# TtesseractT/Synthetic-Audio-Detection

Measured on AMD Instinct MI355X. Metric: 4s@32kHz segments/sec end-to-end (mel+ResNet+ensemble), 1/2/4/8 MI355X, higher is better.
Workload: dtype bf16; 1 GPU; end-to-end inference: B int16 4 s segments resident in HBM -> mel front end -> ResNet-18@512x512 -> 6 binary heads -> merge (+RCCL all-gather of logits); heads=6, distinct_backbones=1, micro_batch=2048, parallelism=dp1, frontend_overlapped=True

## Files before the change

synthetic-audio-detection_amd/csrc/l2conv.hip:

```cpp
#include "common.hpp"
#include "igemm.hpp"
#include "kernels.hpp"
#include "rwconv.hpp"

namespace sad {

namespace l2c {
constexpr int NW = 4;
constexpr int PW = 18, PR = PW * PW;
constexpr int NDP = (PR + 7) / 8;
constexpr int PATCH = NDP * 1024;
constexpr int ROWB = PW * 128;
constexpr int QP = (NDP + NW - 1) / NW;
constexpr int RESB = 256 * 256;
constexpr int NRP = RESB / 1024 / NW;
constexpr int NDS = 256 * 128 / 1024 / NW;
constexpr int OFF_RES = 2 * PATCH;
constexpr int SMEM_RES = OFF_RES + RESB;
constexpr int NS = 36;
constexpr int NSC = 18;
constexpr int DQ = 4;
constexpr int WV = 8;
constexpr int BAD = 0x7FFFFFF0;
constexpr uint64_t KEY = 0xd92dad912240ull;
constexpr int TABB = NW * QP * 256;
constexpr int TAIL = 512 + TABB;
constexpr int ESH = 27;
static_assert(SMEM_RES + TAIL <= 160 * 1024, "LDS budget");
static_assert(PATCH % 128 == 0 && OFF_RES % 256 == 0, "buffer offsets commute with the chunk XORs");
}

__device__ __forceinline__ int l2c_key(int x) { return (int)((l2c::KEY >> (3 * x)) & 7); }

template <bool RES, bool DS, bool X3, bool ST, bool AB>
__device__ __forceinline__ void l2conv_body(const BlockConvArgs& a) {
  static_assert(!(RES && DS) && !(X3 && DS), "one shortcut form");
  static_assert(!ST || (!RES && !DS && !X3), "statistics: the plain bf16 form");
  static_assert(!AB || (!X3 && !ST), "ablations: the bf16 forms");
  using namespace l2c;
  constexpr int TP = X3 ? 8 : 16;
  constexpr int UPT = 2 * TP;
  constexpr int NUC = 9 * UPT;
  constexpr int PDIV = X3 ? 8 : 16;
  constexpr int DQ = X3 ? 8 : l2c::DQ;
  constexpr int OFF_B = RES || DS ? SMEM_RES : OFF_RES;
  constexpr int OFF_T = OFF_B + 512;
  extern __shared__ __attribute__((aligned(256))) char smem[];
  const int tid = threadIdx.x, lane = tid & 63;
  const int wave = __builtin_amdgcn_readfirstlane(tid >> 6);
  const int fr = lane & 15, fg = lane >> 4;
  const int ab = AB ? a.ablate : 0;
  const int cw = X3 ? (wave & 1) * 32 : wave * 32;
  const int r0w = X3 ? (wave >> 1) * 8 : 0;
  const int w = xcd_remap(blockIdx.x, gridDim.x);
  const int tiles_x = a.W / 16, tiles_img = tiles_x * (a.H / 16);
  const int tiles_p = a.N * tiles_img;
  const int tp_begin = (int)((int64_t)w * tiles_p / gridDim.x), tp_end = (int)((int64_t)(w + 1) * tiles_p / gridDim.x);
  if (tp_begin >= tp_end) {
    if constexpr (ST) a.st_part[(int64_t)w * 256 + tid] = 0.f;
    return;
  }

  l1b_v4 rx = {(unsigned)(uintptr_t)a.in0, (unsigned)((uintptr_t)a.in0 >> 32) & 0xFFFFu, (unsigned)a.in0_bytes, 0x00020000u};
  asm volatile("" : "+s"(rx));
  const void* const rrp = RES ? (const void*)a.res : (const void*)a.in1;
  l1b_v4 rr = {(unsigned)(uintptr_t)rrp, (unsigned)((uintptr_t)rrp >> 32) & 0xFFFFu,
               (unsigned)(RES ? a.res_bytes : a.in1_bytes), 0x00020000u};
  if constexpr (RES || DS) asm volatile("" : "+s"(rr));
  const __amdgpu_buffer_rsrc_t ro =
      __builtin_amdgcn_make_buffer_rsrc((void*)a.out, (short)0, (int)a.out_bytes, 0x00020000);
  const unsigned lds0 = (unsigned)(uintptr_t)(__attribute__((address_space(3))) char*)smem;
  const int ps = (int)a.in0_pstride * 2;
  const int pso = (int)a.out_pstride * 2;
  const int pss = RES ? (int)a.res_pstride * 2 : DS ? a.ss1 * (int)a.in1_pstride * 2 : 0;
  const int srow = RES ? a.W * pss : DS ? a.ss1 * a.W1 * (int)a.in1_pstride * 2 : 0;
  const int orow = a.W * pso;

  struct TileO {
    int base, oy0, ox0, sbase, obase;
  };
  auto tile_o = [&](int t) __attribute__((always_inline)) {
    const int b = t / tiles_img, rem = t - b * tiles_img;
    const int ty = rem / tiles_x;
    TileO o;
    o.oy0 = ty * 16;
    o.ox0 = (rem - ty * tiles_x) * 16;
    o.base = ((b * a.H + o.oy0) * a.W + o.ox0) * ps;
    o.obase = ((b * a.H + o.oy0) * a.W + o.ox0) * pso;
    o.sbase = RES  ? ((b * a.H + o.oy0) * a.W + o.ox0) * pss
              : DS ? ((b * a.H1 + o.oy0 * a.ss1) * a.W1 + o.ox0 * a.ss1) * (int)(a.in1_pstride * 2)
                   : 0;
    return o;
  };
  const int wrap_i = 15 * a.W * ps, wrap_o = 15 * orow, wrap_s = 16 * srow - a.W * pss;
  auto tile_step = [&](const TileO& o) __attribute__((always_inline)) {
    TileO n;
    n.ox0 = o.ox0 + 16;
    n.oy0 = o.oy0;
    n.base = o.base + 16 * ps;
    n.obase = o.obase + 16 * pso;
    n.sbase = o.sbase + 16 * pss;
    if (n.ox0 == a.W) {
      n.ox0 = 0;
      n.oy0 += 16;
      n.base += wrap_i;
      n.obase += wrap_o;
      n.sbase += wrap_s;
      if (n.oy0 == a.H) n.oy0 = 0;
    }
    return n;
  };

  const int TA = (int)lds0 + OFF_T + (wave * (QP * 64) + lane) * 4;
  auto piece_entry = [&](int k) __attribute__((always_inline)) {
    const int r = 8 * (wave + NW * k) + (lane >> 3);
    const int Y = (r * 3641) >> 16, X = r - PW * Y;
    const int edge = (r >= PR ? 1 : 0) | (Y == 0 ? 2 : 0) | (Y == PW - 1 ? 4 : 0) | (X == 0 ? 8 : 0) | (X == PW - 1 ? 16 : 0);
    const unsigned off = (unsigned)((Y * a.W + X) * ps + (((lane & 7) ^ l2c_key(X)) << 4)) >> 4;
    return (int)(((unsigned)edge << ESH) | (off & ((1u << ESH) - 1)));
  };
  auto patch_base = [&](const TileO& o) __attribute__((always_inline)) { return o.base - (a.W + 1) * ps; };
  auto patch_mask = [&](const TileO& o) __attribute__((always_inline)) {
    return (int)((unsigned)(1 | (o.oy0 == 0 ? 2 : 0) | (o.oy0 + 16 == a.H ? 4 : 0) | (o.ox0 == 0 ? 8 : 0) |
                            (o.ox0 + 16 == a.W ? 16 : 0))
                 << ESH);
  };
  const unsigned dstw = __builtin_amdgcn_readfirstlane(lds0 + wave * 1024);
  auto issue_piece = [&](auto kc, auto cc, int e, int pbase, int pmask) __attribute__((always_inline)) {
    constexpr int k = decltype(kc)::value, c = decltype(cc)::value;
    if constexpr (NW * k + NW - 1 >= NDP)
      if (wave + NW * k >= NDP) return;
    l1b_dma16<c * PATCH + k * NW * 1024>(rx, (e & pmask) ? BAD : pbase + (int)((unsigned)e << 4), dstw);
  };
  const int pxr = 4 * wave + (lane >> 4);
  const int RV = pxr * pss + (((lane & 15) ^ pxr) << 4);
  auto issue_res = [&](auto kc, const TileO& o) __attribute__((always_inline)) {
    constexpr int k = decltype(kc)::value;
    l1b_dma16<OFF_RES + k * NW * 1024>(rr, RV + (o.sbase + k * srow), dstw);
  };
  const int pxd = 8 * (wave & 1) + (lane >> 3);
  const int DV = (wave >> 1) * srow + pxd * pss + (((lane & 7) ^ ((pxd >> 1) & 7)) << 4);
  auto issue_ds = [&](auto kc, const TileO& o) __attribute__((always_inline)) {
    constexpr int k = decltype(kc)::value;
    l1b_dma16<OFF_RES + k * NW * 1024>(rr, DV + (o.sbase + 2 * k * srow), dstw);
  };
  l1b_v4 wds[2][2];
  if constexpr (DS) {
#pragma unroll
    for (int i = 0; i < 2; ++i)
#pragma unroll
      for (int h = 0; h < 2; ++h)
        wds[i][h] = *(const l1b_v4*)((const u16*)a.wt + (size_t)(cw + 16 * i + fr) * a.wt_ld + 9 * 128 + (fg + 4 * h) * 8);
  }

  l1b_v4 wr[2][NS];
#pragma unroll
  for (int i = 0; i < 2; ++i)
#pragma unroll
    for (int s = 0; s < NS; ++s) {
      const int c = s / NSC, tap = (s % NSC) >> 1, h = s & 1;
      wr[i][s] = *(const l1b_v4*)((const u16*)a.wt + (size_t)(cw + 16 * i + fr) * a.wt_ld + tap * 128 + c * 64 +
                                  (fg + 4 * h) * 8);
    }
  if (tid < (X3 ? 16 : 32)) *(float4*)(smem + OFF_B + 16 * tid) = *(const float4*)(a.bias + 4 * tid);
  TileO ocur = tile_o(tp_begin);
  l1b_for<QP>([&](auto kc) __attribute__((always_inline)) {
    constexpr int k = decltype(kc)::value;
    const int e = piece_entry(k);
    l1b_st<int>(TA + 256 * k, e);
    issue_piece(kc, std::integral_constant<int, 0>{}, e, patch_base(ocur), patch_mask(ocur));
  });

  int I2[3];
#pragma unroll
  for (int kx = 0; kx < 3; ++kx)
    I2[kx] = (int)lds0 + r0w * ROWB + (fr + kx) * 128 + ((fg ^ l2c_key(fr + kx)) << 4);
  const int BA = (int)lds0 + OFF_B + (cw + fg * 4) * 4;
  const int OV = ((r0w + (fg & 1)) * a.W + fr) * pso + ((X3 ? 64 * (cw >> 5) : cw) + (fg >> 1) * 8) * 2;
  const int RB = (int)lds0 + OFF_RES + (r0w * 16 + fr) * 256 + ((((X3 ? 8 * (cw >> 5) : cw >> 3) + (fg >> 1)) ^ fr) << 4) +
                 (fg & 1) * 8;
  const int DD = (int)lds0 + OFF_RES + fr * 128 + ((fg ^ ((fr >> 1) & 7)) << 4);
  const int rl = a.relu ? 0 : (int)0x80008000u;
  const bool relu = a.relu;

  asm volatile("s_waitcnt vmcnt(0)" ::: "memory");
  __syncthreads();
  f32x4 acc[2][TP];
#pragma unroll
  for (int i = 0; i < 2; ++i) {
    const f32x4 b0 = l1b_ld<f32x4>(BA + 64 * i);
#pragma unroll
    for (int j = 0; j < TP; ++j) acc[i][j] = b0;
  }

  float st_s[2][4] = {}, st_q[2][4] = {};
  for (int t = tp_begin; t < tp_end; ++t) {
    const TileO ostep = tile_step(ocur);
    const TileO onext = t + 1 < tp_end ? ostep : ocur;
    const TileO o = ocur;
    const int pb1 = patch_base(o) + 128, pm1 = patch_mask(o);
    const int pb0n = patch_base(onext), pm0n = patch_mask(onext);

    l1b_for<2>([&](auto cc) __attribute__((always_inline)) {
      constexpr int c = decltype(cc)::value;
      if constexpr (c == 0)
        asm volatile("s_waitcnt vmcnt(16)" ::: "memory");
      else
        asm volatile("s_waitcnt vmcnt(0)" ::: "memory");
      __builtin_amdgcn_s_barrier();
      asm volatile("" ::: "memory");
      int pe = l1b_ld<int>(TA);
      int I2c[3][2];
#pragma unroll
      for (int kx = 0; kx < 3; ++kx) {
        I2c[kx][0] = I2[kx] + c * PATCH;
        I2c[kx][1] = I2c[kx][0] ^ 64;
      }
      auto rd = [&](auto uc) __attribute__((always_inline)) -> l1b_v4 {
        constexpr int u = decltype(uc)::value;
        constexpr int tap = u / UPT, ky = tap / 3, kx = tap % 3;
        constexpr int j = X3 ? (u % UPT) / 2 : u % 16, h = X3 ? u % 2 : (u % UPT) / 16;
        return l1b_ld<l1b_v4>(I2c[kx][h] + (j + ky) * ROWB);
      };
      l1b_v4 bq[DQ];
      l1b_for<DQ>([&](auto uc) __attribute__((always_inline)) { bq[decltype(uc)::value] = rd(uc); });
      l1b_for<NUC>([&](auto uc) __attribute__((always_inline)) {
        constexpr int u = decltype(uc)::value;
        constexpr int tap = u / UPT;
        constexpr int j = X3 ? (u % UPT) / 2 : u % 16, h = X3 ? u % 2 : (u % UPT) / 16;
        constexpr int s = c * NSC + 2 * tap + h;
        constexpr int s_hi = c * NSC + 2 * tap, s_lo = s_hi + 1;
        const l1b_v4 bf = bq[u % DQ];
        if constexpr (u + DQ < NUC) bq[u % DQ] = rd(std::integral_constant<int, u + DQ>{});
        if constexpr (u % PDIV == 0 && u / PDIV < QP) {
          constexpr int k = u / PDIV;
          if (!(ab & 32))
            issue_piece(std::integral_constant<int, k>{}, std::integral_constant<int, c ^ 1>{}, pe, c == 0 ? pb1 : pb0n,
                        c == 0 ? pm1 : pm0n);
          if constexpr (k + 1 < QP) pe = l1b_ld<int>(TA + 256 * (k + 1));
        }
        if constexpr (RES && c == 0 && u % PDIV == PDIV / 2 && u / PDIV < NRP)
          issue_res(std::integral_constant<int, u / PDIV>{}, o);
        if constexpr (DS && c == 0 && u % 32 == 8 && u / 32 < NDS) issue_ds(std::integral_constant<int, u / 32>{}, o);
        auto mm = [&](auto ic, auto sc) __attribute__((always_inline)) {
          constexpr int i = decltype(ic)::value, ss = decltype(sc)::value;
          if constexpr (i == 1 && ss >= NS - WV)
            l1b_mfma_v(acc[i][j], wr[i][ss], bf);
          else
            l1b_mfma_a(acc[i][j], wr[i][ss], bf);
        };
        if constexpr (!X3) {
          mm(std::integral_constant<int, 0>{}, std::integral_constant<int, s>{});
          mm(std::integral_constant<int, 1>{}, std::integral_constant<int, s>{});
        } else if constexpr (u == NUC - 2) {
          const l1b_v4 xl = bq[(u + 1) % DQ];
          static_assert(j == TP - 1 && h == 0, "last fragment");
          if constexpr (s_hi >= NS - WV)
            asm volatile(
                "v_mfma_f32_16x16x32_bf16 %0, %2, %6, %0\n\t"
                "v_mfma_f32_16x16x32_bf16 %1, %3, %6, %1\n\t"
                "v_mfma_f32_16x16x32_bf16 %0, %4, %6, %0\n\t"
                "v_mfma_f32_16x16x32_bf16 %1, %5, %6, %1\n\t"
                "v_mfma_f32_16x16x32_bf16 %0, %2, %7, %0\n\t"
                "v_mfma_f32_16x16x32_bf16 %1, %3, %7, %1\n\t"
                "s_nop 11"
                : "+v"(acc[0][j]), "+v"(acc[1][j])
                : "a"(wr[0][s_hi]), "v"(wr[1][s_hi]), "a"(wr[0][s_lo]), "v"(wr[1][s_lo]), "v"(bf), "v"(xl));
          else
            asm volatile(
                "v_mfma_f32_16x16x32_bf16 %0, %2, %6, %0\n\t"
                "v_mfma_f32_16x16x32_bf16 %1, %3, %6, %1\n\t"
                "v_mfma_f32_16x16x32_bf16 %0, %4, %6, %0\n\t"
                "v_mfma_f32_16x16x32_bf16 %1, %5, %6, %1\n\t"
                "v_mfma_f32_16x16x32_bf16 %0, %2, %7, %0\n\t"
                "v_mfma_f32_16x16x32_bf16 %1, %3, %7, %1\n\t"
                "s_nop 11"
                : "+v"(acc[0][j]), "+v"(acc[1][j])
                : "a"(wr[0][s_hi]), "a"(wr[1][s_hi]), "a"(wr[0][s_lo]), "a"(wr[1][s_lo]), "v"(bf), "v"(xl));
        } else if constexpr (u == NUC - 1) {
        } else if constexpr (h == 0) {
          mm(std::integral_constant<int, 0>{}, std::integral_constant<int, s_hi>{});
          mm(std::integral_constant<int, 1>{}, std::integral_constant<int, s_hi>{});
          mm(std::integral_constant<int, 0>{}, std::integral_constant<int, s_lo>{});
          mm(std::integral_constant<int, 1>{}, std::integral_constant<int, s_lo>{});
        } else {
          mm(std::integral_constant<int, 0>{}, std::integral_constant<int, s_hi>{});
          mm(std::integral_constant<int, 1>{}, std::integral_constant<int, s_hi>{});
        }
      });
    });
    if constexpr (DS) {
      constexpr int DQD = 8;
      const int DD1 = DD ^ 64;
      auto rdd = [&](auto uc) __attribute__((always_inline)) -> l1b_v4 {
        constexpr int u = decltype(uc)::value;
        return l1b_ld<l1b_v4>((u / 16 ? DD1 : DD) + (u % 16) * 16 * 128);
      };
      l1b_v4 bd[DQD];
      l1b_for<DQD>([&](auto uc) __attribute__((always_inline)) { bd[decltype(uc)::value] = rdd(uc); });
      l1b_for<32>([&](auto uc) __attribute__((always_inline)) {
        constexpr int u = decltype(uc)::value, h = u / 16, j = u % 16;
        const l1b_v4 bf = bd[u % DQD];
        if constexpr (u + DQD < 32) bd[u % DQD] = rdd(std::integral_constant<int, u + DQD>{});
        l1b_mfma_v(acc[0][j], wds[0][h], bf);
        l1b_mfma_v(acc[1][j], wds[1][h], bf);
      });
    }
    __builtin_amdgcn_sched_barrier(0);
    asm volatile("s_nop 11" ::: "memory");
    __builtin_amdgcn_sched_barrier(0);
    f32x4 bv[2];
#pragma unroll
    for (int i = 0; i < 2; ++i) bv[i] = l1b_ld<f32x4>(BA + 64 * i);

#pragma unroll
    for (int j = 0; j < TP; j += 2) {
      const int osj = o.obase + j * orow;
#pragma unroll
      for (int i = 0; i < 2; ++i) {
        f32x4 v0 = acc[i][j], v1 = acc[i][j + 1];
        const int rbi = i ? RB ^ 32 : RB;
        if constexpr (X3) {
          if constexpr (RES) {
            const l1b_v2 h0 = l1b_ld<l1b_v2>(rbi + j * 4096);
            const l1b_v2 l0 = l1b_ld<l1b_v2>((rbi ^ 64) + j * 4096);
            const l1b_v2 h1 = l1b_ld<l1b_v2>(rbi + (j + 1) * 4096);
            const l1b_v2 l1 = l1b_ld<l1b_v2>((rbi ^ 64) + (j + 1) * 4096);
            v0[0] += __uint_as_float(h0.x << 16) + __uint_as_float(l0.x << 16);
            v0[1] += __uint_as_float(h0.x & 0xFFFF0000u) + __uint_as_float(l0.x & 0xFFFF0000u);
            v0[2] += __uint_as_float(h0.y << 16) + __uint_as_float(l0.y << 16);
            v0[3] += __uint_as_float(h0.y & 0xFFFF0000u) + __uint_as_float(l0.y & 0xFFFF0000u);
            v1[0] += __uint_as_float(h1.x << 16) + __uint_as_float(l1.x << 16);
            v1[1] += __uint_as_float(h1.x & 0xFFFF0000u) + __uint_as_float(l1.x & 0xFFFF0000u);
            v1[2] += __uint_as_float(h1.y << 16) + __uint_as_float(l1.y << 16);
            v1[3] += __uint_as_float(h1.y & 0xFFFF0000u) + __uint_as_float(l1.y & 0xFFFF0000u);
          }
          if (relu)
#pragma unroll
            for (int r = 0; r < 4; ++r) {
              v0[r] = fmaxf(v0[r], 0.f);
              v1[r] = fmaxf(v1[r], 0.f);
            }
          uint32_t qh[4] = {l1b_pk(v0[0], v0[1]), l1b_pk(v0[2], v0[3]), l1b_pk(v1[0], v1[1]), l1b_pk(v1[2], v1[3])};
          const float vv[8] = {v0[0], v0[1], v0[2], v0[3], v1[0], v1[1], v1[2], v1[3]};
          uint32_t ql[4];
#pragma unroll
          for (int e = 0; e < 4; ++e)
            ql[e] = l1b_pk(vv[2 * e] - __uint_as_float(qh[e] << 16), vv[2 * e + 1] - __uint_as_float(qh[e] & 0xFFFF0000u));
#pragma unroll
          for (int e = 0; e < 2; ++e) {
            const auto rh = __builtin_amdgcn_permlane16_swap(qh[e], qh[e + 2], false, false);
            qh[e] = rh[0];
            qh[e + 2] = rh[1];
            const auto rl2 = __builtin_amdgcn_permlane16_swap(ql[e], ql[e + 2], false, false);
            ql[e] = rl2[0];
            ql[e + 2] = rl2[1];
          }
          __builtin_amdgcn_raw_buffer_store_b128((l1b_v4){qh[0], qh[1], qh[2], qh[3]}, ro, OV + 32 * i, osj, 0);
          __builtin_amdgcn_raw_buffer_store_b128((l1b_v4){ql[0], ql[1], ql[2], ql[3]}, ro, OV + 32 * i + 64, osj, 0);
          acc[i][j] = bv[i];
          acc[i][j + 1] = bv[i];
          continue;
        }
        if constexpr (RES) {
          const l1b_v2 r0 = l1b_ld<l1b_v2>(rbi + j * 4096);
          const l1b_v2 r1 = l1b_ld<l1b_v2>(rbi + (j + 1) * 4096);
          v0[0] += __uint_as_float(r0.x << 16);
          v0[1] += __uint_as_float(r0.x & 0xFFFF0000u);
          v0[2] += __uint_as_float(r0.y << 16);
          v0[3] += __uint_as_float(r0.y & 0xFFFF0000u);
          v1[0] += __uint_as_float(r1.x << 16);
          v1[1] += __uint_as_float(r1.x & 0xFFFF0000u);
          v1[2] += __uint_as_float(r1.y << 16);
          v1[3] += __uint_as_float(r1.y & 0xFFFF0000u);
        }
        if constexpr (ST) {
#pragma unroll
          for (int e = 0; e < 4; ++e) {
            st_s[i][e] += v0[e];
            st_s[i][e] += v1[e];
            st_q[i][e] = fmaf(v0[e], v0[e], st_q[i][e]);
            st_q[i][e] = fmaf(v1[e], v1[e], st_q[i][e]);
          }
        }
        uint32_t q[4] = {l1b_pk(v0[0], v0[1]), l1b_pk(v0[2], v0[3]), l1b_pk(v1[0], v1[1]), l1b_pk(v1[2], v1[3])};
        if constexpr (!ST)
#pragma unroll
          for (int e = 0; e < 4; ++e) q[e] = l1b_relu2s(q[e], rl);
#pragma unroll
        for (int e = 0; e < 2; ++e) {
          const auto r = __builtin_amdgcn_permlane16_swap(q[e], q[e + 2], false, false);
          q[e] = r[0];
          q[e + 2] = r[1];
        }
        if (!(ab & 8)) __builtin_amdgcn_raw_buffer_store_b128((l1b_v4){q[0], q[1], q[2], q[3]}, ro, OV + 32 * i, osj, 0);
        acc[i][j] = bv[i];
        acc[i][j + 1] = bv[i];
      }
    }
    ocur = ostep;
  }
  if constexpr (ST) {
#pragma unroll
    for (int i = 0; i < 2; ++i)
#pragma unroll
      for (int e = 0; e < 4; ++e)
#pragma unroll
        for (int off = 1; off < 16; off <<= 1) {
          st_s[i][e] += __shfl_xor(st_s[i][e], off, 64);
          st_q[i][e] += __shfl_xor(st_q[i][e], off, 64);
        }
    if (fr == 0) {
#pragma unroll
      for (int i = 0; i < 2; ++i)
#pragma unroll
        for (int e = 0; e < 4; ++e) {
          const int c = cw + 16 * i + 4 * fg + e;
          a.st_part[(int64_t)w * 256 + c] = st_s[i][e];
          a.st_part[(int64_t)w * 256 + 128 + c] = st_q[i][e];
        }
    }
  }
  asm volatile("s_waitcnt vmcnt(0)" ::: "memory");
}

template <bool RES, bool DS, bool X3 = false, bool ST = false>
__global__ __launch_bounds__(256, 1) void l2conv_kernel(BlockConvArgs a) {
  l2conv_body<RES, DS, X3, ST, false>(a);
}
template <bool RES, bool DS>
__global__ __launch_bounds__(256, 1) void l2conv_ablate_kernel(BlockConvArgs a) {
  l2conv_body<RES, DS, false, false, true>(a);
}

int launch_l2conv(const BlockConvArgs& a, hipStream_t s, bool x3) {
  using namespace l2c;
  SAD_REQUIRE(a.KH == 3 && a.KW == 3 && a.stride == 1 && a.pad == 1 && !a.pool_out,
              "variant 41/42: 3x3/s1/p1, no pool");
  SAD_REQUIRE(!a.st_part || (!x3 && !a.in1 && !a.res && !a.relu && a.st_rows),
              "variant 41 statistics: the plain bf16 raw conv (no shortcut / residual / ReLU), st_rows set");
  if (x3) {
    SAD_REQUIRE(!a.in1 && a.Cin == 128 && a.Cout == 64 && a.H % 16 == 0 && a.W % 16 == 0 && a.Ho == a.H &&
                    a.Wo == a.W && a.wt_ld >= 9 * 128 && a.wt_ld % 8 == 0 && a.in0_pstride % 64 == 0 &&
                    a.in0_pstride >= 128 && a.out_pstride % 64 == 0 && a.out_pstride >= 128 &&
                    (!a.res || (a.res_pstride % 64 == 0 && a.res_pstride >= 128)) && a.out,
                "variant 42: split-bf16 64 -> 64 logical 3x3/s1/p1 (layer1), 16 x 16 tiles");
    const int64_t tiles = (int64_t)a.N * (a.H / 16) * (a.W / 16);
    if (tiles == 0) return SAD_OK;
    const int64_t g = std::min<int64_t>(tiles, 256);
    BlockConvArgs b = a;
    b.out_bytes = ((int64_t)a.N * a.H * a.W - 1) * a.out_pstride * 2 + 256;
    SAD_REQUIRE(b.out_bytes < (1ll << 31) - 65536, "variant 42: output passes the 32-bit buffer range");
    static bool attr[2] = {false, false};
    const void* kfn = a.res ? (const void*)l2conv_kernel<true, false, true> : (const void*)l2conv_kernel<false, false, true>;
    const int smem = (a.res ? SMEM_RES : OFF_RES) + TAIL;
    if (!attr[a.res ? 1 : 0]) {
      SAD_CHECK_HIP(hipFuncSetAttribute(kfn, hipFuncAttributeMaxDynamicSharedMemorySize, smem));
      attr[a.res ? 1 : 0] = true;
    }
    if (a.res)
      hipLaunchKernelGGL((l2conv_kernel<true, false, true>), dim3((unsigned)g), dim3(256), smem, s, b);
    else
      hipLaunchKernelGGL((l2conv_kernel<false, false, true>), dim3((unsigned)g), dim3(256), smem, s, b);
    SAD_CHECK_HIP(hipGetLastError());
    return SAD_OK;
  }
  SAD_REQUIRE(!a.in1 || (!a.res && a.Cin1 == 64 && a.ss1 == 2 && a.H1 == 2 * a.H && a.W1 == 2 * a.W &&
                         a.in1_pstride % 8 == 0 && a.wt_ld >= 9 * 128 + 64),
              "variant 41: the shortcut is a 1x1/2 downsample of a 64-channel input at twice the size");
  SAD_REQUIRE(a.Cin == 128 && a.Cout == 128, "variant 41: Cin = Cout = 128");
  SAD_REQUIRE(a.H % 16 == 0 && a.W % 16 == 0 && a.Ho == a.H && a.Wo == a.W, "variant 41: image must tile by 16 x 16");
  SAD_REQUIRE(a.wt_ld >= 9 * 128 && a.wt_ld % 8 == 0, "variant 41: weight rows");
  SAD_REQUIRE(a.in0_pstride % 8 == 0 && a.out_pstride % 8 == 0 && (!a.res || a.res_pstride % 8 == 0) &&
                  a.in0_pstride >= 128 && a.out_pstride >= 128 && (!a.res || a.res_pstride >= 128),
              "variant 41: 16-B aligned pixel strides");
  SAD_REQUIRE(a.out, "null output");
  const int64_t tiles = (int64_t)a.N * (a.H / 16) * (a.W / 16);
  if (tiles == 0) return SAD_OK;
  const int64_t g = std::min<int64_t>(tiles, 256);
  BlockConvArgs b = a;
  b.out_bytes = ((int64_t)a.N * a.H * a.W - 1) * a.out_pstride * 2 + 256;
  SAD_REQUIRE(b.out_bytes < (1ll << 31) - 65536, "variant 41: output passes the 32-bit buffer range");
  auto go = [&](auto kern, int smem, bool& attr) {
    if (!attr) {
      SAD_CHECK_HIP(hipFuncSetAttribute((const void*)kern, hipFuncAttributeMaxDynamicSharedMemorySize, smem));
      attr = true;
    }
    hipLaunchKernelGGL(kern, dim3((unsigned)g), dim3(256), smem, s, b);
    return SAD_OK;
  };
  static bool attr[7] = {};
  int rc;
  if (a.st_part) {
    rc = go(l2conv_kernel<false, false, false, true>, OFF_RES + TAIL, attr[6]);
    if (rc == SAD_OK) *a.st_rows = (int)g;
  } else if (a.res) {
    rc = a.ablate ? go(l2conv_ablate_kernel<true, false>, SMEM_RES + TAIL, attr[3])
                  : go(l2conv_kernel<true, false>, SMEM_RES + TAIL, attr[0]);
  } else if (a.in1) {
    rc = a.ablate ? go(l2conv_ablate_kernel<false, true>, SMEM_RES + TAIL, attr[4])
                  : go(l2conv_kernel<false, true>, SMEM_RES + TAIL, attr[1]);
  } else {
    rc = a.ablate ? go(l2conv_ablate_kernel<false, false>, OFF_RES + TAIL, attr[5])
                  : go(l2conv_kernel<false, false>, OFF_RES + TAIL, attr[2]);
  }
  if (rc != SAD_OK) return rc;
  SAD_CHECK_HIP(hipGetLastError());
  return SAD_OK;
}

}
```

synthetic-audio-detection_amd/csrc/l2s2conv.hip:

```cpp
#include "common.hpp"
#include "igemm.hpp"
#include "kernels.hpp"
#include "rwconv.hpp"

namespace sad {

namespace l2s {
constexpr int NW = 4;
constexpr int PRR = 17, PCW = 33;
constexpr int NEV = 9;
constexpr int PXB = 128;
constexpr int ROWB = PCW * PXB;
constexpr int ODDC = 17 * PXB;
constexpr int NPX = PRR * PCW;
constexpr int NDP = (NPX * PXB + 1023) / 1024;
constexpr int PATCH = NDP * 1024;
constexpr int QP = (NDP + NW - 1) / NW;
constexpr int OFF_BIAS = 2 * PATCH;
constexpr int SMEM = OFF_BIAS + 512;
constexpr int NS = 18;
constexpr int TP = 8;
constexpr int NUC = 9 * 2 * TP;
constexpr int DQ = 8;
constexpr int PDIV = 8;
constexpr int BAD = 0x7FFFFFF0;
constexpr uint64_t KEY = 0x7929284ef1797ull;
static_assert(SMEM <= 160 * 1024, "LDS budget");
static_assert(NUC / PDIV >= QP, "pieces fit the chunk's units");
static_assert(NW - 1 + NW * (QP - 2) < NDP, "only the last piece index can pass the patch");
static_assert(8 * ROWB + ODDC + 16 * PXB <= 65535, "fragment offsets are ds_read immediates");
}

__device__ __forceinline__ int l2s_key(int x) { return (int)((l2s::KEY >> (3 * x)) & 7); }

template <bool ST = false>
__global__ __launch_bounds__(256, 1) void l2s2conv_kernel(BlockConvArgs a) {
  using namespace l2s;
  const int ab = a.ablate;
  extern __shared__ __attribute__((aligned(16))) char smem[];
  const int tid = threadIdx.x, lane = tid & 63;
  const int wave = __builtin_amdgcn_readfirstlane(tid >> 6);
  const int fr = lane & 15, fg = lane >> 4;
  const int cw = wave * 32;
  const int w = xcd_remap(blockIdx.x, gridDim.x);
  const int tiles_x = a.Wo / 16, tiles_img = tiles_x * (a.Ho / 16);
  const int tiles_p = a.N * tiles_img;
  const int tp_begin = (int)((int64_t)w * tiles_p / gridDim.x), tp_end = (int)((int64_t)(w + 1) * tiles_p / gridDim.x);
  if (tp_begin >= tp_end) {
    if constexpr (ST) a.st_part[(int64_t)w * 256 + tid] = 0.f;
    return;
  }

  const __amdgpu_buffer_rsrc_t rx =
      __builtin_amdgcn_make_buffer_rsrc((void*)a.in0, (short)0, (int)a.in0_bytes, 0x00020000);
  const __amdgpu_buffer_rsrc_t ro =
      __builtin_amdgcn_make_buffer_rsrc((void*)a.out, (short)0, (int)a.out_bytes, 0x00020000);
  const unsigned lds0 = (unsigned)(uintptr_t)(__attribute__((address_space(3))) char*)smem;
  const int ps = (int)a.in0_pstride * 2;

  struct TileO {
    int base, b, oy0, ox0;
  };
  auto tile_o = [&](int t) __attribute__((always_inline)) {
    const int b = t / tiles_img, rem = t - b * tiles_img;
    const int ty = rem / tiles_x;
    TileO o;
    o.b = b;
    o.oy0 = ty * 16;
    o.ox0 = (rem - ty * tiles_x) * 16;
    o.base = ((b * a.H + 2 * o.oy0) * a.W + 2 * o.ox0) * ps;
    return o;
  };
  int prel[QP];
#pragma unroll
  for (int k = 0; k < QP; ++k) {
    const int u = 8 * (wave + NW * k) + (lane >> 3);
    const int r = (u * 1986) >> 16;
    const int cu = u - PCW * r;
    const int Y = r < NEV ? 2 * r : 2 * (r - NEV) + 1;
    const bool odd = cu >= 17;
    const int xp = odd ? cu - 17 : cu;
    const int X = 2 * xp + (odd ? 1 : 0);
    const int c = (lane & 7) ^ l2s_key(xp);
    prel[k] = (((Y - 1) * a.W + (X - 1)) * ps + (c << 4)) | (Y == 0 ? 1 : 0) | (X == 0 ? 2 : 0) | (u >= NPX ? 4 : 0);
  }
  const int hstep = 16 * a.W * ps;
  auto issue_piece = [&](int k, const TileO& o, int h) __attribute__((always_inline)) {
    const int q = wave + NW * k;
    if (k == QP - 1 && q >= NDP) return;
    const int mask = 4 | (h == 0 && o.oy0 == 0 ? 1 : 0) | (o.ox0 == 0 ? 2 : 0);
    const int e = prel[k];
    const int off = o.base + h * hstep + (e & ~15);
    dma16_m0(rx, (e & mask) ? BAD : off, lds0 + h * PATCH + q * 1024);
  };

  l1b_v4 wr[2][NS];
#pragma unroll
  for (int i = 0; i < 2; ++i)
#pragma unroll
    for (int s = 0; s < NS; ++s)
      wr[i][s] = *(const l1b_v4*)((const u16*)a.wt + (size_t)(cw + 16 * i + fr) * a.wt_ld + (s >> 1) * 64 +
                                  (s & 1) * 32 + fg * 8);
  if (tid < 32) *(float4*)(smem + OFF_BIAS + 16 * tid) = *(const float4*)(a.bias + 4 * tid);
  auto biasv = [&](int i) __attribute__((always_inline)) {
    return *(const f32x4*)(smem + OFF_BIAS + (cw + 16 * i + fg * 4) * 4);
  };
  {
    const TileO o0 = tile_o(tp_begin);
#pragma unroll
    for (int k = 0; k < QP; ++k) issue_piece(k, o0, 0);
  }
  asm volatile("s_waitcnt vmcnt(0)" ::: "memory");
  __syncthreads();
  f32x4 acc[2][TP];
#pragma unroll
  for (int i = 0; i < 2; ++i) {
    const f32x4 b0 = biasv(i);
#pragma unroll
    for (int j = 0; j < TP; ++j) acc[i][j] = b0;
  }

  int L[3][2];
#pragma unroll
  for (int kx = 0; kx < 3; ++kx) {
    const int xp = fr + (kx == 2 ? 1 : 0);
    const int key = l2s_key(xp);
#pragma unroll
    for (int kh = 0; kh < 2; ++kh) L[kx][kh] = (kx == 1 ? ODDC : 0) + xp * PXB + (((4 * kh + fg) ^ key) << 4);
  }

  float st_s[2][4] = {}, st_q[2][4] = {};
  for (int t = tp_begin; t < tp_end; ++t) {
    const TileO o = tile_o(t);
    const TileO onext = tile_o(t + 1 < tp_end ? t + 1 : t);
    const int frt = fr, fgt = fg;
    const int obase = ((o.b * a.Ho + o.oy0) * a.Wo + o.ox0) * (int)(a.out_pstride * 2);

    l1b_for<2>([&](auto hc) __attribute__((always_inline)) {
      constexpr int h = decltype(hc)::value;
      asm volatile("s_waitcnt vmcnt(8)" ::: "memory");
      __builtin_amdgcn_s_barrier();
      asm volatile("" ::: "memory");
      int B[3][2][2];
#pragma unroll
      for (int kx = 0; kx < 3; ++kx)
#pragma unroll
        for (int kh = 0; kh < 2; ++kh)
#pragma unroll
          for (int p = 0; p < 2; ++p) B[kx][kh][p] = L[kx][kh] + h * PATCH + p * NEV * ROWB;
      auto rd = [&](auto uc) __attribute__((always_inline)) -> uint4 {
        constexpr int u = decltype(uc)::value;
        constexpr int tap = u / 16, ky = tap / 3, kx = tap % 3, kh = (u / 8) & 1, j = u % 8;
        constexpr int p = ky == 1 ? 1 : 0, row = ky == 1 ? j : j + ky / 2;
        return *(const uint4*)(smem + B[kx][kh][p] + row * ROWB);
      };
      uint4 bq[DQ];
      l1b_for<DQ>([&](auto uc) __attribute__((always_inline)) { bq[decltype(uc)::value] = rd(uc); });
      l1b_for<NUC>([&](auto uc) __attribute__((always_inline)) {
        constexpr int u = decltype(uc)::value;
        constexpr int s = 2 * (u / 16) + ((u / 8) & 1), j = u % 8;
        const uint4 bf = bq[u % DQ];
        if constexpr (u + DQ < NUC) bq[u % DQ] = rd(std::integral_constant<int, u + DQ>{});
        if constexpr (u % PDIV == 0 && u / PDIV < QP) {
          if (ab & 32) {
          } else if constexpr (h == 0)
            issue_piece(u / PDIV, o, 1);
          else
            issue_piece(u / PDIV, onext, 0);
        }
        l1b_mfma_a(acc[0][j], wr[0][s], bf);
        l1b_mfma_a(acc[1][j], wr[1][s], bf);
      });
      __builtin_amdgcn_sched_barrier(0);
      asm volatile("s_nop 11" ::: "memory");
      __builtin_amdgcn_sched_barrier(0);

#pragma unroll
      for (int j = 0; j < TP; j += 2) {
#pragma unroll
        for (int i = 0; i < 2; ++i) {
          const f32x4 v0 = acc[i][j], v1 = acc[i][j + 1];
          if constexpr (ST) {
#pragma unroll
            for (int e = 0; e < 4; ++e) {
              st_s[i][e] += v0[e];
              st_s[i][e] += v1[e];
              st_q[i][e] = fmaf(v0[e], v0[e], st_q[i][e]);
              st_q[i][e] = fmaf(v1[e], v1[e], st_q[i][e]);
            }
          }
          uint32_t q[4] = {l1b_pk(v0[0], v0[1]), l1b_pk(v0[2], v0[3]), l1b_pk(v1[0], v1[1]), l1b_pk(v1[2], v1[3])};
          if (a.relu)
#pragma unroll
            for (int e = 0; e < 4; ++e) q[e] = l1b_relu2(q[e]);
#pragma unroll
          for (int e = 0; e < 2; ++e) {
            const auto r = __builtin_amdgcn_permlane16_swap(q[e], q[e + 2], false, false);
            q[e] = r[0];
            q[e + 2] = r[1];
          }
          const int px = (8 * h + j + (fgt & 1)) * a.Wo + frt;
          const int co = cw + 16 * i + (fgt >> 1) * 8;
          if (!(ab & 8))
            __builtin_amdgcn_raw_buffer_store_b128(__builtin_bit_cast(l1b_v4, make_uint4(q[0], q[1], q[2], q[3])),
                                                   ro, px * (int)(a.out_pstride * 2) + co * 2, obase, 0);
          const f32x4 b0 = biasv(i);
          acc[i][j] = b0;
          acc[i][j + 1] = b0;
        }
      }
    });
  }
  if constexpr (ST) {
#pragma unroll
    for (int i = 0; i < 2; ++i)
#pragma unroll
      for (int e = 0; e < 4; ++e)
#pragma unroll
        for (int off = 1; off < 16; off <<= 1) {
          st_s[i][e] += __shfl_xor(st_s[i][e], off, 64);
          st_q[i][e] += __shfl_xor(st_q[i][e], off, 64);
        }
    if (fr == 0) {
#pragma unroll
      for (int i = 0; i < 2; ++i)
#pragma unroll
        for (int e = 0; e < 4; ++e) {
          const int c = cw + 16 * i + 4 * fg + e;
          a.st_part[(int64_t)w * 256 + c] = st_s[i][e];
          a.st_part[(int64_t)w * 256 + 128 + c] = st_q[i][e];
        }
    }
  }
  asm volatile("s_waitcnt vmcnt(0)" ::: "memory");
}

int launch_l2s2conv(const BlockConvArgs& a, hipStream_t s) {
  using namespace l2s;
  SAD_REQUIRE(a.KH == 3 && a.KW == 3 && a.stride == 2 && a.pad == 1 && !a.in1 && !a.res && !a.pool_out,
              "variant 43: 3x3/s2/p1, no shortcut, residual or pool");
  SAD_REQUIRE(!a.st_part || (!a.relu && a.st_rows), "variant 43 statistics: the raw conv (no ReLU), st_rows set");
  SAD_REQUIRE(a.Cin == 64 && a.Cout == 128, "variant 43: Cin 64, Cout 128");
  SAD_REQUIRE(a.Ho % 16 == 0 && a.Wo % 16 == 0 && a.H == 2 * a.Ho && a.W == 2 * a.Wo,
              "variant 43: output must tile by 16 x 16, input twice its size");
  SAD_REQUIRE(a.wt_ld >= 9 * 64 && a.wt_ld % 8 == 0, "variant 43: weight rows");
  SAD_REQUIRE(a.in0_pstride % 8 == 0 && a.in0_pstride >= 64 && a.out_pstride % 8 == 0 && a.out_pstride >= 128 && a.out,
              "variant 43: 16-B aligned pixel strides, an output");
  const int64_t tiles = (int64_t)a.N * (a.Ho / 16) * (a.Wo / 16);
  if (tiles == 0) return SAD_OK;
  const int64_t g = std::min<int64_t>(tiles, 256);
  BlockConvArgs b = a;
  b.out_bytes = ((int64_t)a.N * a.Ho * a.Wo - 1) * a.out_pstride * 2 + 256;
  SAD_REQUIRE(b.out_bytes < (1ll << 31) - 65536, "variant 43: output passes the 32-bit buffer range");
  if (a.st_part) {
    static bool attr = false;
    if (!attr) {
      SAD_CHECK_HIP(hipFuncSetAttribute((const void*)l2s2conv_kernel<true>, hipFuncAttributeMaxDynamicSharedMemorySize, SMEM));
      attr = true;
    }
    hipLaunchKernelGGL(l2s2conv_kernel<true>, dim3((unsigned)g), dim3(256), SMEM, s, b);
    *a.st_rows = (int)g;
  } else {
    static bool attr = false;
    if (!attr) {
      SAD_CHECK_HIP(hipFuncSetAttribute((const void*)l2s2conv_kernel<false>, hipFuncAttributeMaxDynamicSharedMemorySize, SMEM));
      attr = true;
    }
    hipLaunchKernelGGL(l2s2conv_kernel<false>, dim3((unsigned)g), dim3(256), SMEM, s, b);
  }
  SAD_CHECK_HIP(hipGetLastError());
  return SAD_OK;
}

}
```

Measured before the change: 65980 segments/s.

## Fold bias into first MFMA and stream tile offsets in layer-2 convs

Result: no change. 65840 segments/s (-0.2%).

```diff
diff --git a/synthetic-audio-detection_amd/csrc/l2conv.hip b/synthetic-audio-detection_amd/csrc/l2conv.hip
--- a/synthetic-audio-detection_amd/csrc/l2conv.hip
+++ b/synthetic-audio-detection_amd/csrc/l2conv.hip
@@ -44,6 +44,7 @@
   constexpr int PDIV = X3 ? 8 : 16;
   constexpr int DQ = X3 ? 8 : l2c::DQ;
   constexpr int OFF_B = RES || DS ? SMEM_RES : OFF_RES;
+  constexpr bool CB = !X3 && !RES;
   constexpr int OFF_T = OFF_B + 512;
   extern __shared__ __attribute__((aligned(256))) char smem[];
   const int tid = threadIdx.x, lane = tid & 63;
@@ -186,11 +187,13 @@
   asm volatile("s_waitcnt vmcnt(0)" ::: "memory");
   __syncthreads();
   f32x4 acc[2][TP];
-#pragma unroll
-  for (int i = 0; i < 2; ++i) {
-    const f32x4 b0 = l1b_ld<f32x4>(BA + 64 * i);
-#pragma unroll
-    for (int j = 0; j < TP; ++j) acc[i][j] = b0;
+  if constexpr (!CB) {
+#pragma unroll
+    for (int i = 0; i < 2; ++i) {
+      const f32x4 b0 = l1b_ld<f32x4>(BA + 64 * i);
+#pragma unroll
+      for (int j = 0; j < TP; ++j) acc[i][j] = b0;
+    }
   }
 
   float st_s[2][4] = {}, st_q[2][4] = {};
@@ -200,6 +203,11 @@
     const TileO o = ocur;
     const int pb1 = patch_base(o) + 128, pm1 = patch_mask(o);
     const int pb0n = patch_base(onext), pm0n = patch_mask(onext);
+    f32x4 bv[2];
+    if constexpr (CB) {
+#pragma unroll
+      for (int i = 0; i < 2; ++i) bv[i] = l1b_ld<f32x4>(BA + 64 * i);
+    }
 
     l1b_for<2>([&](auto cc) __attribute__((always_inline)) {
       constexpr int c = decltype(cc)::value;
@@ -244,7 +252,9 @@
         if constexpr (DS && c == 0 && u % 32 == 8 && u / 32 < NDS) issue_ds(std::integral_constant<int, u / 32>{}, o);
         auto mm = [&](auto ic, auto sc) __attribute__((always_inline)) {
           constexpr int i = decltype(ic)::value, ss = decltype(sc)::value;
-          if constexpr (i == 1 && ss >= NS - WV)
+          if constexpr (CB && ss == 0)
+            l1b_mfma_ac(acc[i][j], wr[i][ss], bf, bv[i]);
+          else if constexpr (i == 1 && ss >= NS - WV)
             l1b_mfma_v(acc[i][j], wr[i][ss], bf);
           else
             l1b_mfma_a(acc[i][j], wr[i][ss], bf);
@@ -309,9 +319,10 @@
     __builtin_amdgcn_sched_barrier(0);
     asm volatile("s_nop 11" ::: "memory");
     __builtin_amdgcn_sched_barrier(0);
-    f32x4 bv[2];
-#pragma unroll
-    for (int i = 0; i < 2; ++i) bv[i] = l1b_ld<f32x4>(BA + 64 * i);
+    if constexpr (!CB) {
+#pragma unroll
+      for (int i = 0; i < 2; ++i) bv[i] = l1b_ld<f32x4>(BA + 64 * i);
+    }
 
 #pragma unroll
     for (int j = 0; j < TP; j += 2) {
@@ -394,8 +405,10 @@
           q[e + 2] = r[1];
         }
         if (!(ab & 8)) __builtin_amdgcn_raw_buffer_store_b128((l1b_v4){q[0], q[1], q[2], q[3]}, ro, OV + 32 * i, osj, 0);
-        acc[i][j] = bv[i];
-        acc[i][j + 1] = bv[i];
+        if constexpr (!CB) {
+          acc[i][j] = bv[i];
+          acc[i][j + 1] = bv[i];
+        }
       }
     }
     ocur = ostep;
diff --git a/synthetic-audio-detection_amd/csrc/l2s2conv.hip b/synthetic-audio-detection_amd/csrc/l2s2conv.hip
--- a/synthetic-audio-detection_amd/csrc/l2s2conv.hip
+++ b/synthetic-audio-detection_amd/csrc/l2s2conv.hip
@@ -33,10 +33,11 @@
 
 __device__ __forceinline__ int l2s_key(int x) { return (int)((l2s::KEY >> (3 * x)) & 7); }
 
-template <bool ST = false>
-__global__ __launch_bounds__(256, 1) void l2s2conv_kernel(BlockConvArgs a) {
+template <bool ST, bool AB>
+__device__ __forceinline__ void l2s2conv_body(const BlockConvArgs& a) {
+  static_assert(!(ST && AB), "ablations: the inference form");
   using namespace l2s;
-  const int ab = a.ablate;
+  const int ab = AB ? a.ablate : 0;
   extern __shared__ __attribute__((aligned(16))) char smem[];
   const int tid = threadIdx.x, lane = tid & 63;
   const int wave = __builtin_amdgcn_readfirstlane(tid >> 6);
@@ -51,25 +52,43 @@
     return;
   }
 
-  const __amdgpu_buffer_rsrc_t rx =
-      __builtin_amdgcn_make_buffer_rsrc((void*)a.in0, (short)0, (int)a.in0_bytes, 0x00020000);
+  l1b_v4 rx = {(unsigned)(uintptr_t)a.in0, (unsigned)((uintptr_t)a.in0 >> 32) & 0xFFFFu, (unsigned)a.in0_bytes, 0x00020000u};
+  asm volatile("" : "+s"(rx));
   const __amdgpu_buffer_rsrc_t ro =
       __builtin_amdgcn_make_buffer_rsrc((void*)a.out, (short)0, (int)a.out_bytes, 0x00020000);
   const unsigned lds0 = (unsigned)(uintptr_t)(__attribute__((address_space(3))) char*)smem;
   const int ps = (int)a.in0_pstride * 2;
+  const int pso = (int)a.out_pstride * 2;
+  const int orow = a.Wo * pso;
 
   struct TileO {
-    int base, b, oy0, ox0;
+    int base, obase, oy0, ox0;
   };
   auto tile_o = [&](int t) __attribute__((always_inline)) {
     const int b = t / tiles_img, rem = t - b * tiles_img;
     const int ty = rem / tiles_x;
     TileO o;
-    o.b = b;
     o.oy0 = ty * 16;
     o.ox0 = (rem - ty * tiles_x) * 16;
     o.base = ((b * a.H + 2 * o.oy0) * a.W + 2 * o.ox0) * ps;
+    o.obase = ((b * a.Ho + o.oy0) * a.Wo + o.ox0) * pso;
     return o;
+  };
+  const int wrap_i = 31 * a.W * ps, wrap_o = 15 * orow;
+  auto tile_step = [&](const TileO& o) __attribute__((always_inline)) {
+    TileO n;
+    n.ox0 = o.ox0 + 16;
+    n.oy0 = o.oy0;
+    n.base = o.base + 32 * ps;
+    n.obase = o.obase + 16 * pso;
+    if (n.ox0 == a.Wo) {
+      n.ox0 = 0;
+      n.oy0 += 16;
+      n.base += wrap_i;
+      n.obase += wrap_o;
+      if (n.oy0 == a.Ho) n.oy0 = 0;
+    }
+    return n;
   };
   int prel[QP];
 #pragma unroll
@@ -85,13 +104,16 @@
     prel[k] = (((Y - 1) * a.W + (X - 1)) * ps + (c << 4)) | (Y == 0 ? 1 : 0) | (X == 0 ? 2 : 0) | (u >= NPX ? 4 : 0);
   }
   const int hstep = 16 * a.W * ps;
-  auto issue_piece = [&](int k, const TileO& o, int h) __attribute__((always_inline)) {
-    const int q = wave + NW * k;
-    if (k == QP - 1 && q >= NDP) return;
-    const int mask = 4 | (h == 0 && o.oy0 == 0 ? 1 : 0) | (o.ox0 == 0 ? 2 : 0);
+  auto patch_mask = [&](const TileO& o, int h) __attribute__((always_inline)) {
+    return 4 | (h == 0 && o.oy0 == 0 ? 1 : 0) | (o.ox0 == 0 ? 2 : 0);
+  };
+  const unsigned dstw = __builtin_amdgcn_readfirstlane(lds0 + wave * 1024);
+  auto issue_piece = [&](auto kc, auto hc, int pbase, int pmask) __attribute__((always_inline)) {
+    constexpr int k = decltype(kc)::value, h = decltype(hc)::value;
+    if constexpr (NW * k + NW - 1 >= NDP)
+      if (wave + NW * k >= NDP) return;
     const int e = prel[k];
-    const int off = o.base + h * hstep + (e & ~15);
-    dma16_m0(rx, (e & mask) ? BAD : off, lds0 + h * PATCH + q * 1024);
+    l1b_dma16<h * PATCH + k * NW * 1024>(rx, (e & pmask) ? BAD : pbase + (e & ~15), dstw);
   };
 
   l1b_v4 wr[2][NS];
@@ -102,74 +124,78 @@
       wr[i][s] = *(const l1b_v4*)((const u16*)a.wt + (size_t)(cw + 16 * i + fr) * a.wt_ld + (s >> 1) * 64 +
                                   (s & 1) * 32 + fg * 8);
   if (tid < 32) *(float4*)(smem + OFF_BIAS + 16 * tid) = *(const float4*)(a.bias + 4 * tid);
-  auto biasv = [&](int i) __attribute__((always_inline)) {
-    return *(const f32x4*)(smem + OFF_BIAS + (cw + 16 * i + fg * 4) * 4);
-  };
+  TileO ocur = tile_o(tp_begin);
   {
-    const TileO o0 = tile_o(tp_begin);
-#pragma unroll
-    for (int k = 0; k < QP; ++k) issue_piece(k, o0, 0);
-  }
-  asm volatile("s_waitcnt vmcnt(0)" ::: "memory");
-  __syncthreads();
-  f32x4 acc[2][TP];
-#pragma unroll
-  for (int i = 0; i < 2; ++i) {
-    const f32x4 b0 = biasv(i);
-#pragma unroll
-    for (int j = 0; j < TP; ++j) acc[i][j] = b0;
-  }
-
-  int L[3][2];
+    const int pb = ocur.base, pm = patch_mask(ocur, 0);
+    l1b_for<QP>([&](auto kc) __attribute__((always_inline)) { issue_piece(kc, std::integral_constant<int, 0>{}, pb, pm); });
+  }
+
+  int B[2][3][2][2];
 #pragma unroll
   for (int kx = 0; kx < 3; ++kx) {
     const int xp = fr + (kx == 2 ? 1 : 0);
     const int key = l2s_key(xp);
 #pragma unroll
-    for (int kh = 0; kh < 2; ++kh) L[kx][kh] = (kx == 1 ? ODDC : 0) + xp * PXB + (((4 * kh + fg) ^ key) << 4);
-  }
+    for (int kh = 0; kh < 2; ++kh) {
+      const int L = (kx == 1 ? ODDC : 0) + xp * PXB + (((4 * kh + fg) ^ key) << 4);
+#pragma unroll
+      for (int h = 0; h < 2; ++h)
+#pragma unroll
+        for (int p = 0; p < 2; ++p) {
+          int v = (int)lds0 + L + h * PATCH + p * NEV * ROWB;
+          asm volatile("" : "+v"(v));
+          B[h][kx][kh][p] = v;
+        }
+    }
+  }
+  const int OV = ((fg & 1) * a.Wo + fr) * pso + (cw + (fg >> 1) * 8) * 2;
+  const int rl = a.relu ? 0 : (int)0x80008000u;
+
+  asm volatile("s_waitcnt vmcnt(0)" ::: "memory");
+  __syncthreads();
+  f32x4 bv[2];
+#pragma unroll
+  for (int i = 0; i < 2; ++i) bv[i] = l1b_ld<f32x4>((int)lds0 + OFF_BIAS + (cw + 16 * i + fg * 4) * 4);
+  f32x4 acc[2][TP];
 
   float st_s[2][4] = {}, st_q[2][4] = {};
   for (int t = tp_begin; t < tp_end; ++t) {
-    const TileO o = tile_o(t);
-    const TileO onext = tile_o(t + 1 < tp_end ? t + 1 : t);
-    const int frt = fr, fgt = fg;
-    const int obase = ((o.b * a.Ho + o.oy0) * a.Wo + o.ox0) * (int)(a.out_pstride * 2);
+    const TileO ostep = tile_step(ocur);
+    const TileO onext = t + 1 < tp_end ? ostep : ocur;
+    const TileO o = ocur;
+    const int pb1 = o.base + hstep, pm1 = patch_mask(o, 1);
+    const int pb0n = onext.base, pm0n = patch_mask(onext, 0);
 
     l1b_for<2>([&](auto hc) __attribute__((always_inline)) {
       constexpr int h = decltype(hc)::value;
       asm volatile("s_waitcnt vmcnt(8)" ::: "memory");
       __builtin_amdgcn_s_barrier();
       asm volatile("" ::: "memory");
-      int B[3][2][2];
-#pragma unroll
-      for (int kx = 0; kx < 3; ++kx)
-#pragma unroll
-        for (int kh = 0; kh < 2; ++kh)
-#pragma unroll
-          for (int p = 0; p < 2; ++p) B[kx][kh][p] = L[kx][kh] + h * PATCH + p * NEV * ROWB;
-      auto rd = [&](auto uc) __attribute__((always_inline)) -> uint4 {
+      auto rd = [&](auto uc) __attribute__((always_inline)) -> l1b_v4 {
         constexpr int u = decltype(uc)::value;
         constexpr int tap = u / 16, ky = tap / 3, kx = tap % 3, kh = (u / 8) & 1, j = u % 8;
         constexpr int p = ky == 1 ? 1 : 0, row = ky == 1 ? j : j + ky / 2;
-        return *(const uint4*)(smem + B[kx][kh][p] + row * ROWB);
+        return l1b_ld<l1b_v4>(B[h][kx][kh][p] + row * ROWB);
       };
-      uint4 bq[DQ];
+      l1b_v4 bq[DQ];
       l1b_for<DQ>([&](auto uc) __attribute__((always_inline)) { bq[decltype(uc)::value] = rd(uc); });
       l1b_for<NUC>([&](auto uc) __attribute__((always_inline)) {
         constexpr int u = decltype(uc)::value;
         constexpr int s = 2 * (u / 16) + ((u / 8) & 1), j = u % 8;
-        const uint4 bf = bq[u % DQ];
+        const l1b_v4 bf = bq[u % DQ];
         if constexpr (u + DQ < NUC) bq[u % DQ] = rd(std::integral_constant<int, u + DQ>{});
         if constexpr (u % PDIV == 0 && u / PDIV < QP) {
-          if (ab & 32) {
-          } else if constexpr (h == 0)
-            issue_piece(u / PDIV, o, 1);
-          else
-            issue_piece(u / PDIV, onext, 0);
-        }
-        l1b_mfma_a(acc[0][j], wr[0][s], bf);
-        l1b_mfma_a(acc[1][j], wr[1][s], bf);
+          if (!(ab & 32))
+            issue_piece(std::integral_constant<int, u / PDIV>{}, std::integral_constant<int, h ^ 1>{}, h == 0 ? pb1 : pb0n,
+                        h == 0 ? pm1 : pm0n);
+        }
+        if constexpr (u < TP) {
+          l1b_mfma_ac(acc[0][j], wr[0][s], bf, bv[0]);
+          l1b_mfma_ac(acc[1][j], wr[1][s], bf, bv[1]);
+        } else {
+          l1b_mfma_a(acc[0][j], wr[0][s], bf);
+          l1b_mfma_a(acc[1][j], wr[1][s], bf);
+        }
       });
       __builtin_amdgcn_sched_barrier(0);
       asm volatile("s_nop 11" ::: "memory");
@@ -177,6 +203,7 @@
 
 #pragma unroll
       for (int j = 0; j < TP; j += 2) {
+        const int osj = o.obase + (8 * h + j) * orow;
 #pragma unroll
         for (int i = 0; i < 2; ++i) {
           const f32x4 v0 = acc[i][j], v1 = acc[i][j + 1];
@@ -190,26 +217,20 @@
             }
           }
           uint32_t q[4] = {l1b_pk(v0[0], v0[1]), l1b_pk(v0[2], v0[3]), l1b_pk(v1[0], v1[1]), l1b_pk(v1[2], v1[3])};
-          if (a.relu)
-#pragma unroll
-            for (int e = 0; e < 4; ++e) q[e] = l1b_relu2(q[e]);
+          if constexpr (!ST)
+#pragma unroll
+            for (int e = 0; e < 4; ++e) q[e] = l1b_relu2s(q[e], rl);
 #pragma unroll
           for (int e = 0; e < 2; ++e) {
             const auto r = __builtin_amdgcn_permlane16_swap(q[e], q[e + 2], false, false);
             q[e] = r[0];
             q[e + 2] = r[1];
           }
-          const int px = (8 * h + j + (fgt & 1)) * a.Wo + frt;
-          const int co = cw + 16 * i + (fgt >> 1) * 8;
-          if (!(ab & 8))
-            __builtin_amdgcn_raw_buffer_store_b128(__builtin_bit_cast(l1b_v4, make_uint4(q[0], q[1], q[2], q[3])),
-                                                   ro, px * (int)(a.out_pstride * 2) + co * 2, obase, 0);
-          const f32x4 b0 = biasv(i);
-          acc[i][j] = b0;
-          acc[i][j + 1] = b0;
+          if (!(ab & 8)) __builtin_amdgcn_raw_buffer_store_b128((l1b_v4){q[0], q[1], q[2], q[3]}, ro, OV + 32 * i, osj, 0);
         }
       }
     });
+    ocur = ostep;
   }
   if constexpr (ST) {
 #pragma unroll
@@ -234,6 +255,12 @@
   }
   asm volatile("s_waitcnt vmcnt(0)" ::: "memory");
 }
+
+template <bool ST = false>
+__global__ __launch_bounds__(256, 1) void l2s2conv_kernel(BlockConvArgs a) {
+  l2s2conv_body<ST, false>(a);
+}
+__global__ __launch_bounds__(256, 1) void l2s2conv_ablate_kernel(BlockConvArgs a) { l2s2conv_body<false, true>(a); }
 
 int launch_l2s2conv(const BlockConvArgs& a, hipStream_t s) {
   using namespace l2s;
@@ -252,22 +279,23 @@
   BlockConvArgs b = a;
   b.out_bytes = ((int64_t)a.N * a.Ho * a.Wo - 1) * a.out_pstride * 2 + 256;
   SAD_REQUIRE(b.out_bytes < (1ll << 31) - 65536, "variant 43: output passes the 32-bit buffer range");
-  if (a.st_part) {
-    static bool attr = false;
+  auto go = [&](auto kern, bool& attr) {
     if (!attr) {
-      SAD_CHECK_HIP(hipFuncSetAttribute((const void*)l2s2conv_kernel<true>, hipFuncAttributeMaxDynamicSharedMemorySize, SMEM));
+      SAD_CHECK_HIP(hipFuncSetAttribute((const void*)kern, hipFuncAttributeMaxDynamicSharedMemorySize, SMEM));
       attr = true;
     }
-    hipLaunchKernelGGL(l2s2conv_kernel<true>, dim3((unsigned)g), dim3(256), SMEM, s, b);
-    *a.st_rows = (int)g;
+    hipLaunchKernelGGL(kern, dim3((unsigned)g), dim3(256), SMEM, s, b);
+    return SAD_OK;
+  };
+  static bool attr[3] = {};
+  int rc;
+  if (a.st_part) {
+    rc = go(l2s2conv_kernel<true>, attr[0]);
+    if (rc == SAD_OK) *a.st_rows = (int)g;
   } else {
-    static bool attr = false;
-    if (!attr) {
-      SAD_CHECK_HIP(hipFuncSetAttribute((const void*)l2s2conv_kernel<false>, hipFuncAttributeMaxDynamicSharedMemorySize, SMEM));
-      attr = true;
-    }
-    hipLaunchKernelGGL(l2s2conv_kernel<false>, dim3((unsigned)g), dim3(256), SMEM, s, b);
-  }
+    rc = a.ablate ? go(l2s2conv_ablate_kernel, attr[2]) : go(l2s2conv_kernel<false>, attr[1]);
+  }
+  if (rc != SAD_OK) return rc;
   SAD_CHECK_HIP(hipGetLastError());
   return SAD_OK;
 }
```
